# EricssonResearch/Robust-Tracking-MPC-over-Lossy-Networks

Hardware: AMD Instinct MI355X
Metric: QP solves/sec (= MPC steps/sec) at batch (higher is better)
Workload: dtype f64

## Files before the change

include/tmpc.h:

```cpp
#ifndef TMPC_H
#define TMPC_H

#include <stddef.h>
#include <stdint.h>

#ifdef __cplusplus
extern "C" {
#endif

#define TMPC_ABI_VERSION 5

#define TMPC_OK            0
#define TMPC_E_INVALID    -1
#define TMPC_E_UNSUPPORTED -2
#define TMPC_E_DEVICE     -3
#define TMPC_E_NOMEM      -4

#define TMPC_STATUS_OPTIMAL     0
#define TMPC_STATUS_MAX_ITER    1
#define TMPC_STATUS_INFEASIBLE  2
#define TMPC_STATUS_NUMERICAL   3
#define TMPC_STATUS_UNBOUNDED   4

typedef struct tmpc_problem {
// ... 128 lines not shown
                         int32_t *not_optimal, int32_t *overrun, int32_t *age_max, int64_t *age_sum, int32_t *iters_max, int64_t *iters_sum,
                         double *e_sum, double *e_max, double *e_q, float *kernel_ms);
int tmpc_series_stats(int device, int64_t B, int32_t T, const double *e, const uint32_t *word, int32_t G, const int32_t *group, int32_t n_q,
                      const double *q, int32_t *n_alive, int32_t *n_nan, int32_t *lost_up, int32_t *lost_down, int32_t *adopted, int32_t *tube,
                      int32_t *not_optimal, int32_t *overrun, int32_t *age_max, int64_t *age_sum, int32_t *iters_max, int64_t *iters_sum,
                      double *e_sum, double *e_max, double *e_q, float *kernel_ms);
int tmpc_mc_get_physics_error(tmpc_handle *h, int64_t B, double *err2_phys);

#define TMPC_ACTUATOR_CONSISTENT 0
#define TMPC_ACTUATOR_SMART      1
int tmpc_mc_set_actuator(tmpc_handle *h, int kind);

int tmpc_synchronize(tmpc_handle *h);

int tmpc_set_call_overlap(tmpc_handle *h, int on);
int tmpc_debug_lane_counters(tmpc_handle *h, int64_t *calls_per_lane, int64_t *cross_lane_waits, int reset);
int tmpc_debug_calls_conflict(int32_t nx, int32_t nu, int32_t N, int64_t B_a, const void *const *a, int64_t B_b, const void *const *b);

int tmpc_last_kernel_ms(tmpc_handle *h, float *ms);

int tmpc_kernel_ms_total(tmpc_handle *h, float *total_ms, int32_t *launches, int reset);

int tmpc_get_dims(const tmpc_handle *h, int variant, int32_t *nv, int32_t *nc, int32_t *npar);
int tmpc_get_factoring(const tmpc_handle *h, int variant, int32_t *nd, int32_t *ncc, int32_t *kc);

int tmpc_get_condensed(const tmpc_handle *h, int variant,
                       double *H, double *F1, double *F2, double *G, double *g0, double *E);

int tmpc_lp_batch(int device, int32_t d, int32_t nr, const double *H, const double *h,
                  int64_t B, const double *C, const int32_t *relax, double relax_by,
                  double *val, double *x, int32_t *status, int32_t *iters);
// ... 82 lines not shown
```

robust-tracking-mpc-over-lossy-networks_amd/LinearMPCOverNetworks/_native.py:

```python
from __future__ import annotations

import ctypes as C
import os

import numpy as np

_PKG = os.path.dirname(os.path.dirname(os.path.abspath(__file__)))
LIB_PATH = os.environ.get("TMPC_LIB") or os.path.join(_PKG, "lib", "libtmpc_hip.so")
ABI_VERSION = 5

_PTR_FIELDS = ["A", "B", "Q", "R", "P", "T", "K", "K_anc",
               "Hx", "hx", "Hu", "hu", "HT", "hT", "HZ", "hZ", "HZW", "hZW", "HTP", "hTP"]
_INT_FIELDS = ["nx", "nu", "N", "rx", "ru", "rT", "rZ", "rZW",
               "fixed_x0", "extended", "literal_terminal_row", "max_iter"]

_dp = C.POINTER(C.c_double)
_ip = C.POINTER(C.c_int32)
_up = C.POINTER(C.c_uint8)


class TmpcProblem(C.Structure):
    _fields_ = ([(n, C.c_int32) for n in _INT_FIELDS] + [("tol", C.c_double)]
                + [(n, _dp) for n in _PTR_FIELDS] + [("rTP", C.c_int32), ("terminal_equality", C.c_int32)])

# ... 133 lines not shown
        L.tmpc_lp_batch.restype = C.c_int
        L.tmpc_order_statistics.argtypes = [C.c_int, C.c_int64, C.c_int32, C.c_void_p, C.c_int32, C.c_void_p, C.c_void_p, C.c_void_p]
        L.tmpc_order_statistics.restype = C.c_int
        L.tmpc_estimate_w.argtypes = ([C.c_int, C.c_int32, C.c_int32] + [C.c_void_p] * 3 + [C.c_int, C.c_void_p, C.c_int32, C.c_int64, C.c_int32]
                                      + [C.c_void_p] * 3 + [C.c_uint64, C.c_int64, C.c_int32, C.c_void_p, C.c_double] + [C.c_void_p] * 10)
        L.tmpc_estimate_w.restype = C.c_int
        L.tmpc_estimate_w_models.argtypes = ([C.c_int, C.c_int32, C.c_int32] + [C.c_void_p] * 3 + [C.c_int, C.c_void_p, C.c_void_p, C.c_int32, C.c_int64, C.c_int32]
                                             + [C.c_void_p] * 3 + [C.c_uint64, C.c_int64, C.c_int32, C.c_void_p, C.c_double] + [C.c_void_p] * 10)
        L.tmpc_estimate_w_models.restype = C.c_int
        L.tmpc_synchronize.argtypes = [C.c_void_p]
        L.tmpc_synchronize.restype = C.c_int
        L.tmpc_set_call_overlap.argtypes = [C.c_void_p, C.c_int]
        L.tmpc_set_call_overlap.restype = C.c_int
        L.tmpc_debug_lane_counters.argtypes = [C.c_void_p, C.POINTER(C.c_int64), C.POINTER(C.c_int64), C.c_int]
        L.tmpc_debug_lane_counters.restype = C.c_int
        L.tmpc_debug_calls_conflict.argtypes = [C.c_int32, C.c_int32, C.c_int32, C.c_int64, C.POINTER(C.c_void_p), C.c_int64, C.POINTER(C.c_void_p)]
        L.tmpc_debug_calls_conflict.restype = C.c_int
        L.tmpc_last_kernel_ms.argtypes = [C.c_void_p, C.POINTER(C.c_float)]
        L.tmpc_last_kernel_ms.restype = C.c_int
        L.tmpc_kernel_ms_total.argtypes = [C.c_void_p, C.POINTER(C.c_float), _ip, C.c_int]
        L.tmpc_kernel_ms_total.restype = C.c_int
        L.tmpc_get_dims.argtypes = [C.c_void_p, C.c_int, _ip, _ip, _ip]
        L.tmpc_get_dims.restype = C.c_int
        L.tmpc_get_factoring.argtypes = [C.c_void_p, C.c_int, _ip, _ip, _ip]
        L.tmpc_get_factoring.restype = C.c_int
        L.tmpc_get_condensed.argtypes = [C.c_void_p, C.c_int, _dp, _dp, _dp, _dp, _dp, _dp]
        L.tmpc_get_condensed.restype = C.c_int
        L.tmpc_create_regulator.argtypes = [C.POINTER(TmpcRegulatorProblem), C.c_int, C.POINTER(C.c_void_p)]
        L.tmpc_create_regulator.restype = C.c_int
        L.tmpc_reg_run.argtypes = ([C.c_void_p, C.c_int64, C.c_int32] + [C.c_void_p] * 4 + [C.c_int32] + [C.c_void_p] * 2
# ... 233 lines not shown
        raise RuntimeError(h.error())


def set_call_overlap(h: Handle, on: bool = True):
    if lib().tmpc_set_call_overlap(h.ptr, int(bool(on))) != 0:
        raise RuntimeError(h.error())


def lane_counters(h: Handle, reset: bool = False):
    calls, waits = (C.c_int64 * 2)(), C.c_int64()
    if lib().tmpc_debug_lane_counters(h.ptr, calls, C.byref(waits), int(reset)) != 0:
        raise RuntimeError(h.error())
    return (int(calls[0]), int(calls[1])), int(waits.value)


SOLVE_POINTERS = ("x_k", "ref", "variant", "u_nom", "x_nom0", "xu_ss", "x_nom", "status", "iters")


def calls_conflict(nx: int, nu: int, N: int, B_a: int, a: dict, B_b: int, b: dict) -> bool:
    pa = (C.c_void_p * 9)(*[a.get(k) for k in SOLVE_POINTERS])
    pb = (C.c_void_p * 9)(*[b.get(k) for k in SOLVE_POINTERS])
    rc = lib().tmpc_debug_calls_conflict(nx, nu, N, int(B_a), pa, int(B_b), pb)
    if rc < 0:
        raise RuntimeError("tmpc_debug_calls_conflict: invalid argument")
    return bool(rc)


def last_kernel_ms(h: Handle) -> float:
    ms = C.c_float()
    if lib().tmpc_last_kernel_ms(h.ptr, C.byref(ms)) != 0:
# ... 942 lines not shown
```

robust-tracking-mpc-over-lossy-networks_amd/csrc/tmpc_api.cpp:

```cpp
#include "tmpc_host.hpp"

using namespace tmpc_host;

namespace {

constexpr size_t LANE_SPARE_EVENTS = 64;

template <class T>
int upload(tmpc_handle *h, Variant &v, const T *src, size_t n, const T **dst) {
    void *p = nullptr;
    if (h->device < 0) {
        p = std::malloc((n ? n : 1) * sizeof(T));
        if (!p) { h->err = "out of memory"; return TMPC_E_NOMEM; }
        v.dev.push_back(p);
        v.dev_bytes.push_back(n * sizeof(T));
        if (n) std::memcpy(p, src, n * sizeof(T));
        *dst = static_cast<const T *>(p);
        return TMPC_OK;
    }
    HIP_TRY(h, hipMalloc(&p, (n ? n : 1) * sizeof(T)));
    v.dev.push_back(p);
    v.dev_bytes.push_back(n * sizeof(T));
    if (n) HIP_TRY(h, hipMemcpy(p, src, n * sizeof(T), hipMemcpyHostToDevice));
    *dst = static_cast<const T *>(p);
// ... 274 lines not shown
}

int upload_variant(tmpc_handle *h, Variant &v, const tmpc_problem &p) {
    int rc;
    if ((rc = upload_wave(h, v, p))) return rc;
    if ((rc = upload_block(h, v, p))) return rc;
    if (!v.wave_ok && v.tiles == 0) {
        char buf[200];
        std::snprintf(buf, sizeof buf, "condensed QP (nv=%d, rows=%d) is outside the compiled kernels (nv <= 128)", v.c.nv, v.c.nc);
        h->err = buf;
        return TMPC_E_UNSUPPORTED;
    }
    return TMPC_OK;
}

int join_lanes(tmpc_handle *h) {
    Lane &second = h->lane[1];
    if (second.stream && !second.inflight.empty()) HIP_TRY(h, hipStreamWaitEvent(h->stream, second.inflight.back().end, 0));
    h->cur = 0;
    return TMPC_OK;
}

int ensure_block_ws(tmpc_handle *h, Lane &lane) {
    if (lane.blk_ws.p) return TMPC_OK;
    int ncp = 0, occ_max = 1;
    for (int k = 0; k < h->nvariants; ++k)
        if (h->v[k].tiles) { ncp = std::max(ncp, h->v[k].bq.ncp); occ_max = std::max(occ_max, tmpc::block_occupancy(h->v[k].tiles)); }
    h->blk_blocks = h->n_cu * occ_max;
    HIP_TRY(h, lane.blk_ws.reserve(static_cast<size_t>(h->blk_blocks) * tmpc::block_workspace_rows() * ncp * sizeof(double), lane.stream));
    return TMPC_OK;
}

size_t layout_staging(tmpc_handle *h, int64_t B) {
    const size_t nx = h->nx, nu = h->nu, N = h->N, b = static_cast<size_t>(B);
    auto up = [](size_t v) { return (v + 255) / 256 * 256; };
    h->off_r = up(b * nx * sizeof(double));
    h->off_var = h->off_r + up(b * nx * sizeof(double));
// ... 31 lines not shown
        h->stage_pin = nullptr;
        (void)hipGetLastError();
    }
    (void)layout_staging(h, B);
    return TMPC_OK;
}

int create_lane(tmpc_handle *h, Lane &lane) {
    HIP_TRY(h, hipStreamCreateWithFlags(&lane.stream, hipStreamNonBlocking));
    lane.wc.size = 4096;
    HIP_TRY(h, hipMalloc(reinterpret_cast<void **>(&lane.wc.ring), lane.wc.size * sizeof(unsigned long long)));
    HIP_TRY(h, hipMemset(lane.wc.ring, 0, lane.wc.size * sizeof(unsigned long long)));
    return TMPC_OK;
}

void prune_finished(Lane &lane) {
    while (!lane.inflight.empty()) {
        if (hipEventQuery(lane.inflight.front().end) != hipSuccess) { (void)hipGetLastError(); break; }
        lane.inflight.pop_front();
    }
}

bool conflicts_with_lane(const Lane &lane, const tmpc::CallRanges &call) {
    for (const Lane::InFlight &f : lane.inflight)
        if (tmpc::calls_conflict(f.touched, call)) return true;
    return false;
}

int pick_lane(tmpc_handle *h, const tmpc::CallRanges &call, Lane **out) {
    *out = &h->lane[0];
    if (!h->overlap) return TMPC_OK;
    for (Lane &l : h->lane) prune_finished(l);
    Lane &prev = h->lane[h->cur], &other = h->lane[1 - h->cur];
    if (conflicts_with_lane(prev, call)) {
        if (other.stream && conflicts_with_lane(other, call)) {
            HIP_TRY(h, hipStreamWaitEvent(prev.stream, other.inflight.back().end, 0));
            ++h->lane_waits;
        }
        *out = &prev;
        return TMPC_OK;
    }
    if (!other.stream) {
        if (prev.inflight.empty()) { *out = &prev; return TMPC_OK; }
        if (const int rc = create_lane(h, other)) return rc;
    }
    *out = &other;
    return TMPC_OK;
}

int note_in_flight(tmpc_handle *h, Lane &lane, const tmpc::CallRanges &call) {
    hipEvent_t end = h->ev1;
    if (h->pool_used >= 4096) {
        while (lane.inflight.size() >= LANE_SPARE_EVENTS) {
            HIP_TRY(h, hipEventSynchronize(lane.inflight.front().end));
            lane.inflight.pop_front();
        }
        if (lane.spare.size() < LANE_SPARE_EVENTS) {
            hipEvent_t e = nullptr;
            HIP_TRY(h, hipEventCreateWithFlags(&e, hipEventDisableTiming));
            lane.spare.push_back(e);
        }
        end = lane.spare[lane.spare_next++ % LANE_SPARE_EVENTS];
        HIP_TRY(h, hipEventRecord(end, lane.stream));
    }
    lane.inflight.push_back({call, end});
    ++lane.calls;
    h->cur = static_cast<int>(&lane - h->lane);
    return TMPC_OK;
}

int setup_handle(tmpc_handle *h, const tmpc_problem &p, int device) {
    if (device < 0) {
        for (int k = 0; k < h->nvariants; ++k) {
            const int rc = upload_variant(h, h->v[k], p);
            if (rc == TMPC_E_UNSUPPORTED) h->err.clear();
            else if (rc) return rc;
        }
        return TMPC_OK;
    }
    hipDeviceProp_t prop;
    hipError_t e = hipSetDevice(device);
    if (e == hipSuccess) e = hipGetDeviceProperties(&prop, device);
    if (e != hipSuccess) {
        h->err = std::string("tmpc_create: no usable HIP device: ") + hipGetErrorString(e);
        return TMPC_E_DEVICE;
    }
    h->n_cu = prop.multiProcessorCount;
    if (const int rc = create_lane(h, h->lane[0])) return rc;
    h->stream = h->lane[0].stream;
    for (int i = 0; i < 256; ++i) {
        hipEvent_t a = nullptr, b = nullptr;
        HIP_TRY(h, hipEventCreate(&a));
        HIP_TRY(h, hipEventCreate(&b));
        h->pool.emplace_back(a, b);
    }
    for (int k = 0; k < h->nvariants; ++k)
        if (const int rc = upload_variant(h, h->v[k], p)) return rc;
    return TMPC_OK;
}

template <class Condense>
int create_handle(const char *who, int nx, int nu, int N, int device, tmpc_handle **out, Condense condense) {
    *out = nullptr;
    if (nx <= 0 || nu <= 0 || N <= 0 || nx > 16) {
        g_create_error = std::string(who) + ": need 0 < nx <= 16, nu > 0, N > 0";
        return TMPC_E_INVALID;
    }
    tmpc_handle *h = new (std::nothrow) tmpc_handle();
    if (!h) { g_create_error = "out of memory"; return TMPC_E_NOMEM; }
    h->device = device; h->nx = nx; h->nu = nu; h->N = N;
    int rc = TMPC_E_INVALID;
    try {
// ... 46 lines not shown
                if (v.dev[i] == q) { n = v.dev_bytes[i]; break; }
        std::fwrite(&n, 8, 1, f);
        if (n) std::fwrite(q, 1, n, f);
    }
    std::fclose(f);
    return TMPC_OK;
}

}

namespace tmpc_host {

thread_local std::string g_create_error;

hipError_t sync_lanes(tmpc_handle *h) {
    hipError_t e = h->stream ? hipStreamSynchronize(h->stream) : hipSuccess;
    Lane &second = h->lane[1];
    if (e == hipSuccess && second.stream) e = hipStreamSynchronize(second.stream);
    if (e == hipSuccess)
        for (Lane &l : h->lane) l.inflight.clear();
    return e;
}

int pick_call_lane(tmpc_handle *h, const tmpc::CallRanges &call, Lane **out) { return pick_lane(h, call, out); }
int note_call(tmpc_handle *h, Lane &lane, const tmpc::CallRanges &call) { return h->overlap ? note_in_flight(h, lane, call) : (++lane.calls, TMPC_OK); }

bool use_block(const tmpc_handle *h, const Variant &v) { return h->kernel_path == TMPC_PATH_BLOCK ? v.tiles != 0 : !v.wave_ok; }

int ensure_reg_zero(tmpc_handle *h, int64_t B) {
    const size_t bytes = static_cast<size_t>(B) * h->nx * sizeof(double);
    if (bytes <= h->reg_zero.cap) return TMPC_OK;
    HIP_TRY(h, sync_lanes(h));
    HIP_TRY(h, h->reg_zero.reserve(bytes, h->stream));
    HIP_TRY(h, hipMemset(h->reg_zero.p, 0, bytes));
    return TMPC_OK;
}

int begin_timed_launch(tmpc_handle *h, Lane &lane) {
    hipEvent_t e0 = h->pool.back().first, e1 = h->pool.back().second;
    if (h->pool_used < 4096) {
// ... 161 lines not shown
}

int tmpc_solve_batch_device(tmpc_handle *h, int64_t B, const double *x_k, const double *ref, const uint8_t *variant,
                            double *u_nom, double *x_nom0, double *xu_ss, double *x_nom, int32_t *status, int32_t *iters) {
    if (const int rc = check_solve(h, "tmpc_solve_batch_device", B, x_k, ref, variant, u_nom, xu_ss, status, iters, false); rc || B == 0) return rc;
    if (h->regulator) {
        const int rz = ensure_reg_zero(h, B);
        if (rz) return rz;
        ref = h->reg_zero.as<double>();
    }
    const tmpc::CallRanges call = tmpc::solve_call_ranges(B, h->nx, h->nu, h->N, x_k, h->regulator ? nullptr : ref, variant, u_nom, x_nom0, xu_ss,
                                                          x_nom, status, iters);
    Lane *lane = nullptr;
    if (const int rc = pick_lane(h, call, &lane)) return rc;
    if (const int rc = enqueue(h, *lane, {B, x_k, ref, variant, u_nom, x_nom0, xu_ss, x_nom, status, iters})) return rc;
    return h->overlap ? note_in_flight(h, *lane, call) : (++lane->calls, TMPC_OK);
}

int tmpc_solve_batch(tmpc_handle *h, int64_t B, const double *x_k, const double *ref, const uint8_t *variant,
                     double *u_nom, double *x_nom0, double *xu_ss, double *x_nom, int32_t *status, int32_t *iters) {
    int rc = check_solve(h, "tmpc_solve_batch", B, x_k, ref, variant, u_nom, xu_ss, status, iters, true);
    if (rc || B == 0) return rc;
    if ((rc = join_lanes(h))) return rc;
    if ((rc = ensure_staging(h, B))) return rc;
    if (h->regulator && (rc = ensure_reg_zero(h, B))) return rc;
    const size_t nx = h->nx, nu = h->nu, N = h->N, b = static_cast<size_t>(B);
    const struct { size_t off; const void *host; size_t bytes; } in[] = {
        {0, x_k, b * nx * sizeof(double)}, {h->off_r, h->regulator ? nullptr : ref, b * nx * sizeof(double)}, {h->off_var, variant, b}};
    const struct { size_t off; void *host; size_t bytes; } out[] = {
        {0, u_nom, b * N * nu * sizeof(double)}, {h->off_x0, x_nom0, b * nx * sizeof(double)}, {h->off_ss, xu_ss, b * (nx + nu) * sizeof(double)},
        {h->off_st, status, b * sizeof(int32_t)}, {h->off_it, iters, b * sizeof(int32_t)}, {h->off_xn, x_nom, b * (N + 1) * nx * sizeof(double)}};
// ... 21 lines not shown
        if (a.host) HIP_TRY(h, hipMemcpyAsync(dev_in + a.off, a.host, a.bytes, hipMemcpyHostToDevice, h->stream));
    if ((rc = launch())) return rc;
    for (const auto &a : out)
        if (a.host) HIP_TRY(h, hipMemcpyAsync(a.host, dev_out + a.off, a.bytes, hipMemcpyDeviceToHost, h->stream));
    HIP_TRY(h, sync_lanes(h));
    return TMPC_OK;
}

int tmpc_set_kernel_path(tmpc_handle *h, int path) {
    if (!h || session_bars(h, "tmpc_set_kernel_path")) return TMPC_E_INVALID;
    if (path != TMPC_PATH_AUTO && path != TMPC_PATH_WAVE && path != TMPC_PATH_BLOCK) { h->err = "tmpc_set_kernel_path: unknown path"; return TMPC_E_INVALID; }
    for (int k = 0; k < h->nvariants; ++k) {
        if (path == TMPC_PATH_WAVE && !h->v[k].wave_ok && h->device >= 0) { h->err = "tmpc_set_kernel_path: no wave-per-QP shape covers this problem"; return TMPC_E_UNSUPPORTED; }
        if (path == TMPC_PATH_BLOCK && h->v[k].tiles == 0 && h->device >= 0) { h->err = "tmpc_set_kernel_path: the block kernel needs nv <= 128"; return TMPC_E_UNSUPPORTED; }
    }
    h->kernel_path = path;
    return TMPC_OK;
}

int tmpc_get_kernel_path(const tmpc_handle *h, int variant) {
    if (!h || variant < 0 || variant >= h->nvariants) return TMPC_E_INVALID;
    return use_block(h, h->v[variant]) ? TMPC_PATH_BLOCK : TMPC_PATH_WAVE;
}

int tmpc_debug_dump_layout(const tmpc_handle *h, int variant, const char *path) {
    if (!h || !path || variant < 0 || variant >= h->nvariants) return TMPC_E_INVALID;
    if (h->device >= 0) return TMPC_E_UNSUPPORTED;
    const Variant &v = h->v[variant];
    if (!v.wave_ok) return TMPC_E_UNSUPPORTED;
    const int32_t shp[6] = {v.shape.nvp, v.shape.dp, v.shape.ds, v.shape.kcp, v.shape.cp, v.shape.cs};
// ... 48 lines not shown

int tmpc_set_call_overlap(tmpc_handle *h, int on) {
    if (!h || session_bars(h, "tmpc_set_call_overlap")) return TMPC_E_INVALID;
    if (h->device >= 0 && (on != 0) != (h->overlap != 0)) {
        HIP_TRY(h, hipSetDevice(h->device));
        if (on) HIP_TRY(h, sync_lanes(h));
        else if (const int rc = join_lanes(h)) return rc;
    }
    h->overlap = on ? 1 : 0;
    return TMPC_OK;
}

int tmpc_debug_lane_counters(tmpc_handle *h, int64_t *calls_per_lane, int64_t *cross_lane_waits, int reset) {
    if (!h) return TMPC_E_INVALID;
    if (calls_per_lane)
        for (int k = 0; k < 2; ++k) calls_per_lane[k] = h->lane[k].calls;
    if (cross_lane_waits) *cross_lane_waits = h->lane_waits;
    if (reset) { h->lane[0].calls = h->lane[1].calls = 0; h->lane_waits = 0; }
    return TMPC_OK;
}

int tmpc_debug_calls_conflict(int32_t nx, int32_t nu, int32_t N, int64_t B_a, const void *const *a, int64_t B_b, const void *const *b) {
    if (!a || !b || nx <= 0 || nu <= 0 || N <= 0) return TMPC_E_INVALID;
    const tmpc::CallRanges ra = tmpc::solve_call_ranges(B_a, nx, nu, N, a[0], a[1], a[2], a[3], a[4], a[5], a[6], a[7], a[8]);
    const tmpc::CallRanges rb = tmpc::solve_call_ranges(B_b, nx, nu, N, b[0], b[1], b[2], b[3], b[4], b[5], b[6], b[7], b[8]);
    return tmpc::calls_conflict(ra, rb) ? 1 : 0;
}

int tmpc_last_kernel_ms(tmpc_handle *h, float *ms) {
    if (!h || !ms) return TMPC_E_INVALID;
    if (!h->timed) { h->err = "tmpc_last_kernel_ms: no solve has been enqueued yet"; return TMPC_E_INVALID; }
    HIP_TRY(h, hipEventSynchronize(h->ev1));
    HIP_TRY(h, hipEventElapsedTime(ms, h->ev0, h->ev1));
    return TMPC_OK;
}

int tmpc_kernel_ms_total(tmpc_handle *h, float *total_ms, int32_t *launches, int reset) {
    if (!h) return TMPC_E_INVALID;
    if (h->device < 0) { h->err = "host-only handle"; return TMPC_E_DEVICE; }
    HIP_TRY(h, sync_lanes(h));
    float sum = 0.f;
    size_t busy = 0;
    for (size_t i = 0; i < h->pool_used; ++i) {
        float ms = 0.f;
        HIP_TRY(h, hipEventElapsedTime(&ms, h->pool[i].first, h->pool[i].second));
        if (i > 0 && h->pool_lane[i] != h->pool_lane[busy]) {
            float past = 0.f;
            HIP_TRY(h, hipEventElapsedTime(&past, h->pool[busy].second, h->pool[i].second));
            if (past <= 0.f) continue;
            ms = std::min(ms, past);
        }
        busy = i;
        sum += ms;
    }
    if (total_ms) *total_ms = sum;
    if (launches) *launches = static_cast<int32_t>(h->pool_used);
    if (reset) h->pool_used = 0;
    return TMPC_OK;
}

#ifdef TMPC_STAMPS
int tmpc_debug_stamps(tmpc_handle *h, int variant, long long *out12 ) {
    if (!h || !out12) return TMPC_E_INVALID;
    HIP_TRY(h, sync_lanes(h));
    const long long *src = use_block(h, h->v[variant]) ? h->v[variant].db.dbg : h->v[variant].d.dbg;
    HIP_TRY(h, hipMemcpy(out12, src, 16 * sizeof(long long), hipMemcpyDeviceToHost));
    return TMPC_OK;
}
#endif
// ... 35 lines not shown
```

robust-tracking-mpc-over-lossy-networks_amd/csrc/tmpc_hazard.hpp:

```cpp
#pragma once
#include <cstddef>
#include <cstdint>

namespace tmpc {

struct ByteRange {
    uintptr_t lo = 0, hi = 0;
};

inline bool ranges_overlap(const ByteRange &a, const ByteRange &b) {
    return a.lo < a.hi && b.lo < b.hi && a.lo < b.hi && b.lo < a.hi;
}

struct CallRanges {
    static constexpr int NR = 8, NW = 8;
    ByteRange reads[NR], writes[NW];
    ByteRange hull;
};

inline ByteRange byte_range(const void *p, size_t bytes) {
    ByteRange r;
    if (p != nullptr && bytes != 0) { r.lo = reinterpret_cast<uintptr_t>(p); r.hi = r.lo + bytes; }
    return r;
}
// ... 21 lines not shown
    for (const ByteRange &r : c.writes) grow(r);
    return c;
}

inline bool calls_conflict(const CallRanges &earlier, const CallRanges &later) {
    if (!ranges_overlap(earlier.hull, later.hull)) return false;
    for (const ByteRange &w : earlier.writes) {
        for (const ByteRange &r : later.reads) if (ranges_overlap(w, r)) return true;
        for (const ByteRange &w2 : later.writes) if (ranges_overlap(w, w2)) return true;
    }
    for (const ByteRange &r : earlier.reads)
        for (const ByteRange &w2 : later.writes) if (ranges_overlap(r, w2)) return true;
    return false;
}

}
```

robust-tracking-mpc-over-lossy-networks_amd/csrc/tmpc_host.hpp:

```cpp
#pragma once
#include <hip/hip_runtime.h>

#include <cmath>
#include <cstdio>
#include <cstdlib>
#include <algorithm>
#include <cstdint>
#include <cstring>
#include <deque>
#include <initializer_list>
#include <new>
#include <string>
#include <vector>

#include "tmpc_condense.hpp"
#include "tmpc_device.hpp"
#include "tmpc_hazard.hpp"
#include "tmpc_law.hpp"

namespace tmpc_host __attribute__((visibility("hidden"))) {

struct DeviceBuffer {
    char *p = nullptr;
    size_t cap = 0;
// ... 59 lines not shown
    long long *tick_sum = nullptr, *tick_max = nullptr;
    int64_t tick_B = 0;
    double *err2_phys = nullptr;
    int64_t phys_B = 0;
    int fused = 0;
    std::vector<int32_t> link;
    int64_t link_B = 0;
    double *ser_e = nullptr;
    uint32_t *ser_w = nullptr;
    int64_t ser_B = 0;
    int ser_T = 0;
    tmpc::LawLoop law{};
    int64_t law_B = 0;
};

struct Lane {
    hipStream_t stream = nullptr;
    tmpc::WorkCounter wc;
    DeviceBuffer blk_ws;
    DeviceBuffer save;
    DeviceBuffer ticks;
    struct InFlight {
        tmpc::CallRanges touched;
        hipEvent_t end;
    };
    std::deque<InFlight> inflight;
    std::vector<hipEvent_t> spare;
    size_t spare_next = 0;
    int64_t calls = 0;
};

struct McSession {
    bool open = false, failed = false;
    int64_t B = 0;
    int T = 0, t = 0, extended = 0;
    tmpc::McModel m{};
    tmpc::McState st{};
    tmpc::McExternal ext{};
    int32_t *ws[2] = {nullptr, nullptr};
    bool warm = false;
    std::vector<double> ref;
    bool full_ref = false;
    double *ref_stage = nullptr;
    hipEvent_t ev_in = nullptr, ev_out = nullptr;
// ... 40 lines not shown
};
struct LawState;
struct SensState;
}

struct tmpc_handle {
    int device = 0;
    int n_cu = 0;
    int nvariants = 0;
    int nx = 0, nu = 0, N = 0;
    tmpc_host::Variant v[2];
    bool regulator = false;
    int reg_tube = 0;
    std::vector<double> hA, hB, hK, hKanc, hQ, hR;
    int kernel_path = TMPC_PATH_AUTO;
    tmpc_host::Lane lane[2];
    hipStream_t stream = nullptr;
    int overlap = 1;
    int cur = 0;
    int64_t lane_waits = 0;
    hipEvent_t ev0 = nullptr, ev1 = nullptr;
    bool timed = false;
    std::vector<std::pair<hipEvent_t, hipEvent_t>> pool;
    std::vector<uint8_t> pool_lane;
    size_t pool_used = 0;
    int blk_blocks = 0;
    int want_ticks = 0;
    int ticks_lane = 0;
    int64_t ticks_n = 0;
    tmpc_host::DeviceBuffer reg_zero;
    std::string err;
    tmpc_host::DeviceBuffer stage_dev;
    char *stage_pin = nullptr;
    size_t stage_in_bytes = 0, stage_out_bytes = 0, stage_out_core = 0;
// ... 18 lines not shown
            (h)->err = std::string(#expr) + ": " + hipGetErrorString(e_);                  \
            return TMPC_E_DEVICE;                                                          \
        }                                                                                  \
    } while (0)

extern thread_local std::string g_create_error;

hipError_t sync_lanes(tmpc_handle *h);
bool use_block(const tmpc_handle *h, const Variant &v);
int ensure_reg_zero(tmpc_handle *h, int64_t B);
int begin_timed_launch(tmpc_handle *h, Lane &lane);
int prepare_wave_scratch(tmpc_handle *h, Lane &lane, int64_t B, int nvar);
int enqueue(tmpc_handle *h, Lane &lane, const tmpc::BatchIO &io, int32_t *const *ws = nullptr, bool variants_valid = false);
void release_session(tmpc_handle *h);
int begin_loop(tmpc_handle *h, int64_t B);
bool session_bars(tmpc_handle *h, const char *who);
int pick_call_lane(tmpc_handle *h, const tmpc::CallRanges &call, Lane **out);
int note_call(tmpc_handle *h, Lane &lane, const tmpc::CallRanges &call);
void release_sens(tmpc_handle *h);
bool chol(std::vector<double> &a, int n);
void chol_solve(const std::vector<double> &L, int n, double *x);
std::string spd_inverse(const double *H, int n, std::vector<double> &Hinv);
struct HostModel {
    tmpc::Mat F, Eb, Y, Yp, Rec;
};
std::string host_model(const tmpc_handle *h, int k, HostModel &hm, int &rc);
int sens_signatures(tmpc_handle *h, const char *who, int64_t B, const double *x_k, const double *ref, const uint8_t *variant, const double *u_nom,
                    const double *x_nom0, const double *xu_ss, const int32_t *status, double act_tol, int32_t *flag, int32_t *n_active, uint32_t *active);
void release_law(tmpc_handle *h);
int enqueue_solves(tmpc_handle *h, Lane &lane, const tmpc::BatchIO &io, int32_t *const *ws);
// ... 6 lines not shown
```

robust-tracking-mpc-over-lossy-networks_amd/csrc/tmpc_law.cpp:

```cpp
#include <map>

#include "tmpc_host.hpp"
#include "tmpc_law.hpp"

using namespace tmpc_host;

namespace tmpc_host {

struct LawModel {
    int nv = 0, nc = 0, np = 0, ny = 0, npar = 0;
    std::vector<double> L, Ft, G, F, Eb, g0, Y, Yp, Ep, gp0;
    int nrow() const { return nc + npar; }
    int nrowp() const { return (nrow() + 63) / 64 * 64; }
    int nwords() const { return (nc + 31) / 32; }
};

struct LawRegion {
    std::vector<uint32_t> words;
    std::vector<double> S, K;
};

struct LawKeys {
    std::vector<unsigned long long> key;
    std::vector<int32_t> slot;
// ... 51 lines not shown
    }
    void release_device() {
        for (void *p : {static_cast<void *>(dS), static_cast<void *>(dK), static_cast<void *>(dorder), static_cast<void *>(dhits), static_cast<void *>(dkey),
                        static_cast<void *>(dslot)})
            if (p) (void)hipFree(p);
        dS = dK = nullptr; dorder = nullptr; dhits = nullptr; dkey = nullptr; dslot = nullptr; cap = 0;
    }
};

struct LawState {
    LawVariant v[2];
    double *dAB = nullptr;
    tmpc::LawTable *dtab = nullptr;
    int max_hops = 0;
    unsigned long long *dstats = nullptr;
    DeviceBuffer todo[2];
    DeviceBuffer stage;
};

void release_law(tmpc_handle *h) {
    LawState *s = h->law;
    if (!s) return;
    if (h->device >= 0) {
        for (LawVariant &v : s->v) v.release_device();
        if (s->dAB) (void)hipFree(s->dAB);
        if (s->dtab) (void)hipFree(s->dtab);
        if (s->dstats) (void)hipFree(s->dstats);
        for (DeviceBuffer &b : s->todo) b.release();
        s->stage.release();
    }
    delete s;
// ... 285 lines not shown
        for (int r = first_new; r < static_cast<int>(v.regions.size()); ++r) v.index.erase(v.regions[r].words);
        v.regions.resize(first_new);
        v.rebuild_keys();
        v.order.erase(std::remove_if(v.order.begin(), v.order.end(), [first_new](int32_t id) { return id >= first_new; }), v.order.end());
        for (int64_t i = 0; ids && i < n; ++i)
            if (ids[i] >= first_new) ids[i] = -1;
        if (n_new) *n_new = 0;
    }
    return rc;
}

int quiesce(tmpc_handle *h) {
    if (h->device < 0) return TMPC_OK;
    HIP_TRY(h, hipSetDevice(h->device));
    HIP_TRY(h, sync_lanes(h));
    h->cur = 0;
    return TMPC_OK;
}

struct LawCall {
    int64_t B;
    const double *x_k, *ref;
    const uint8_t *variant;
    const int32_t *hint;
    int max_tries;
    double *u_nom, *x_nom0, *xu_ss, *x_nom;
    int32_t *status, *iters, *region, *tries;
    bool fallback;
    const tmpc::LawLoop *loop = nullptr;
    const uint8_t *skip = nullptr;
    int32_t *const *ws = nullptr;
// ... 84 lines not shown
}

int call_device(tmpc_handle *h, const char *who, const LawCall &c) {
    if (const int rc = check_call(h, who, c); rc || c.B == 0) return rc;
    HIP_TRY(h, hipSetDevice(h->device));
    const tmpc::CallRanges call = law_call_ranges(h, c);
    Lane *lane = nullptr;
    if (const int rc = pick_call_lane(h, call, &lane)) return rc;
    if (const int rc = enqueue_law(h, *lane, who, c)) return rc;
    return note_call(h, *lane, call);
}

int call_host(tmpc_handle *h, const char *who, const LawCall &c) {
    if (const int rc = check_call(h, who, c); rc || c.B == 0) return rc;
    HIP_TRY(h, hipSetDevice(h->device));
    if (Lane &second = h->lane[1]; second.stream && !second.inflight.empty()) HIP_TRY(h, hipStreamWaitEvent(h->stream, second.inflight.back().end, 0));
    h->cur = 0;
    if (const int rc = ensure_state(h, who)) return rc;
    const size_t b = static_cast<size_t>(c.B), nx = h->nx, nu = h->nu, N = h->N, d = sizeof(double);
    struct Part { const void *host_in; void *host_out; size_t bytes; size_t off; };
    Part parts[] = {{c.x_k, nullptr, b * nx * d, 0}, {c.ref, nullptr, b * nx * d, 0}, {c.variant, nullptr, c.variant ? b : 0, 0}, {c.hint, nullptr, c.hint ? b * 4 : 0, 0},
                    {nullptr, c.u_nom, b * N * nu * d, 0}, {nullptr, c.x_nom0, b * nx * d, 0}, {nullptr, c.xu_ss, b * (nx + nu) * d, 0},
                    {nullptr, c.x_nom, c.x_nom ? b * (N + 1) * nx * d : 0, 0}, {nullptr, c.status, b * 4, 0}, {nullptr, c.iters, c.iters ? b * 4 : 0, 0},
                    {nullptr, c.region, b * 4, 0}, {nullptr, c.tries, c.tries ? b * 4 : 0, 0}};
    size_t total = 0;
    for (Part &p : parts) { p.off = total; total += (p.bytes + 255) / 256 * 256; }
    LawState &s = *h->law;
    HIP_TRY(h, s.stage.reserve(std::max<size_t>(total, 256), h->stream));
    char *base = s.stage.p;
    for (const Part &p : parts)
        if (p.host_in && p.bytes) HIP_TRY(h, hipMemcpyAsync(base + p.off, p.host_in, p.bytes, hipMemcpyHostToDevice, h->stream));
    auto at = [&](int i) { return parts[i].bytes ? base + parts[i].off : nullptr; };
// ... 349 lines not shown
```

robust-tracking-mpc-over-lossy-networks_amd/csrc/tmpc_sens.cpp:

```cpp
#include "tmpc_host.hpp"
#include "tmpc_sens.hpp"

using namespace tmpc_host;

namespace tmpc_host {

struct SensModel {
    bool ready = false;
    char *block = nullptr;
    tmpc::SensArgs a{};
};

struct SensState {
    SensModel m[2];
    DeviceBuffer ws[2];
    DeviceBuffer stage;
};

void release_sens(tmpc_handle *h) {
    SensState *s = h->sens;
    if (!s) return;
    for (SensModel &m : s->m)
        if (m.block) (void)hipFree(m.block);
    for (DeviceBuffer &b : s->ws) b.release();
    s->stage.release();
    delete s;
    h->sens = nullptr;
}

bool chol(std::vector<double> &a, int n) {
// ... 271 lines not shown
        a.nz0 = N * nu; a.nz1 = nx; a.nz2 = nx + nu;
        a.Z0 = c.u_nom; a.Z1 = c.x_nom0; a.Z2 = c.xu_ss;
        a.status = c.status; a.variant = c.variant; a.my_variant = k; a.nvariants = h->nvariants;
        a.act_tol = c.act_tol > 0.0 ? c.act_tol : tmpc::SENS_ACT_TOL;
        a.mode = c.mode; a.ybar = c.ybar; a.out = c.out; a.flag = c.flag; a.n_active = c.n_active; a.active = c.active;
        a.nwords = nwords_of(h);
        a.ws = c.mode == tmpc::SENS_MODE_JACOBIAN ? wsbuf.as<double>() : nullptr;
        HIP_TRY(h, tmpc::launch_sens(a, sens_blocks(c.B, h->n_cu, a.nv, a.np), lane.stream));
    }
    HIP_TRY(h, hipEventRecord(h->ev1, lane.stream));
    h->timed = true;
    return TMPC_OK;
}

int primary_behind_secondary(tmpc_handle *h) {
    Lane &second = h->lane[1];
    if (second.stream && !second.inflight.empty()) HIP_TRY(h, hipStreamWaitEvent(h->stream, second.inflight.back().end, 0));
    h->cur = 0;
    return TMPC_OK;
}

tmpc::CallRanges sens_call_ranges(const tmpc_handle *h, const SensCall &c) {
    const size_t b = static_cast<size_t>(c.B), nx = h->nx, nu = h->nu, N = h->N, ny = N * nu + 2 * nx + nu, d = sizeof(double);
    tmpc::CallRanges r;
    static_assert(tmpc::CallRanges::NR >= 8 && tmpc::CallRanges::NW >= 4, "eight arrays read, four written");
    r.reads[0] = tmpc::byte_range(c.x_k, b * nx * d);
    r.reads[1] = tmpc::byte_range(c.ref, b * nx * d);
    r.reads[2] = tmpc::byte_range(c.variant, b);
    r.reads[3] = tmpc::byte_range(c.u_nom, b * N * nu * d);
    r.reads[4] = tmpc::byte_range(c.x_nom0, b * nx * d);
    r.reads[5] = tmpc::byte_range(c.xu_ss, b * (nx + nu) * d);
    r.reads[6] = tmpc::byte_range(c.status, b * sizeof(int32_t));
    r.reads[7] = tmpc::byte_range(c.ybar, b * ny * d);
    r.writes[0] = tmpc::byte_range(c.out, b * (c.mode == tmpc::SENS_MODE_VJP ? 2 * nx : ny * 2 * nx) * d);
// ... 180 lines not shown
```

Measured before the change: 13.00 million.

## Generalize call overlap from two streams to up to four lanes

After: 13.28 million (median of 6 runs). 1.02x the previous value.

```diff
diff --git a/include/tmpc.h b/include/tmpc.h
--- a/include/tmpc.h
+++ b/include/tmpc.h
@@ -166,7 +166,16 @@
 int tmpc_synchronize(tmpc_handle *h);
 
 int tmpc_set_call_overlap(tmpc_handle *h, int on);
+#define TMPC_MAX_LANES 4
+int tmpc_set_call_lanes(tmpc_handle *h, int n);
+int tmpc_get_call_lanes(const tmpc_handle *h);
 int tmpc_debug_lane_counters(tmpc_handle *h, int64_t *calls_per_lane, int64_t *cross_lane_waits, int reset);
+int tmpc_debug_lane_counters_n(tmpc_handle *h, int64_t *calls_per_lane, int64_t *cross_lane_waits, int reset);
+int tmpc_debug_elastic_grid(const tmpc_handle *h, int32_t n_cu, int32_t lanes, int32_t wpb, int64_t B, int32_t *core, int32_t *eligible);
+int tmpc_debug_surplus_yields(uint32_t followers, int32_t lanes);
+int tmpc_debug_plan_lanes(int32_t nx, int32_t nu, int32_t N, int32_t lanes, int32_t n_calls, const int64_t *B, const void *const *ptrs,
+                          int32_t *lane_out, int32_t *waited_out, int32_t *followers_out);
+double tmpc_debug_busy_union(int32_t n, const int32_t *lane, const double *start, const double *end);
 int tmpc_debug_calls_conflict(int32_t nx, int32_t nu, int32_t N, int64_t B_a, const void *const *a, int64_t B_b, const void *const *b);
 
 int tmpc_last_kernel_ms(tmpc_handle *h, float *ms);
diff --git a/robust-tracking-mpc-over-lossy-networks_amd/LinearMPCOverNetworks/_native.py b/robust-tracking-mpc-over-lossy-networks_amd/LinearMPCOverNetworks/_native.py
--- a/robust-tracking-mpc-over-lossy-networks_amd/LinearMPCOverNetworks/_native.py
+++ b/robust-tracking-mpc-over-lossy-networks_amd/LinearMPCOverNetworks/_native.py
@@ -171,6 +171,22 @@
         L.tmpc_set_call_overlap.restype = C.c_int
         L.tmpc_debug_lane_counters.argtypes = [C.c_void_p, C.POINTER(C.c_int64), C.POINTER(C.c_int64), C.c_int]
         L.tmpc_debug_lane_counters.restype = C.c_int
+        if hasattr(L, "tmpc_set_call_lanes"):
+            L.tmpc_set_call_lanes.argtypes = [C.c_void_p, C.c_int]
+            L.tmpc_set_call_lanes.restype = C.c_int
+            L.tmpc_get_call_lanes.argtypes = [C.c_void_p]
+            L.tmpc_get_call_lanes.restype = C.c_int
+            L.tmpc_debug_lane_counters_n.argtypes = [C.c_void_p, C.POINTER(C.c_int64), C.POINTER(C.c_int64), C.c_int]
+            L.tmpc_debug_lane_counters_n.restype = C.c_int
+            L.tmpc_debug_elastic_grid.argtypes = [C.c_void_p, C.c_int32, C.c_int32, C.c_int32, C.c_int64, C.POINTER(C.c_int32), C.POINTER(C.c_int32)]
+            L.tmpc_debug_elastic_grid.restype = C.c_int
+            L.tmpc_debug_surplus_yields.argtypes = [C.c_uint32, C.c_int32]
+            L.tmpc_debug_surplus_yields.restype = C.c_int
+            L.tmpc_debug_plan_lanes.argtypes = [C.c_int32, C.c_int32, C.c_int32, C.c_int32, C.c_int32, C.POINTER(C.c_int64), C.POINTER(C.c_void_p),
+                                                C.POINTER(C.c_int32), C.POINTER(C.c_int32), C.POINTER(C.c_int32)]
+            L.tmpc_debug_plan_lanes.restype = C.c_int
+            L.tmpc_debug_busy_union.argtypes = [C.c_int32, C.POINTER(C.c_int32), C.POINTER(C.c_double), C.POINTER(C.c_double)]
+            L.tmpc_debug_busy_union.restype = C.c_double
         L.tmpc_debug_calls_conflict.argtypes = [C.c_int32, C.c_int32, C.c_int32, C.c_int64, C.POINTER(C.c_void_p), C.c_int64, C.POINTER(C.c_void_p)]
         L.tmpc_debug_calls_conflict.restype = C.c_int
         L.tmpc_last_kernel_ms.argtypes = [C.c_void_p, C.POINTER(C.c_float)]
@@ -434,6 +450,54 @@
     return (int(calls[0]), int(calls[1])), int(waits.value)
 
 
+MAX_LANES = 4
+
+
+def set_call_lanes(h: Handle, n: int):
+    if lib().tmpc_set_call_lanes(h.ptr, int(n)) != 0:
+        raise RuntimeError(h.error())
+
+
+def get_call_lanes(h: Handle) -> int:
+    return int(lib().tmpc_get_call_lanes(h.ptr))
+
+
+def lane_counters_n(h: Handle, reset: bool = False):
+    calls, waits = (C.c_int64 * MAX_LANES)(), C.c_int64()
+    if lib().tmpc_debug_lane_counters_n(h.ptr, calls, C.byref(waits), int(reset)) != 0:
+        raise RuntimeError(h.error())
+    return tuple(int(c) for c in calls), int(waits.value)
+
+
+def elastic_grid(h: Handle, n_cu: int, lanes: int, wpb: int, B: int):
+    core, el = C.c_int32(), C.c_int32()
+    if lib().tmpc_debug_elastic_grid(h.ptr, n_cu, lanes, wpb, int(B), C.byref(core), C.byref(el)) != 0:
+        raise RuntimeError("tmpc_debug_elastic_grid: invalid argument")
+    return int(core.value), bool(el.value)
+
+
+def surplus_yields(followers: int, lanes: int) -> bool:
+    return bool(lib().tmpc_debug_surplus_yields(int(followers), int(lanes)))
+
+
+def plan_lanes(nx: int, nu: int, N: int, lanes: int, calls):
+    n = len(calls)
+    B = (C.c_int64 * max(n, 1))(*[int(b) for b, _ in calls])
+    ptrs = (C.c_void_p * (9 * max(n, 1)))(*[a.get(k) for _, a in calls for k in SOLVE_POINTERS])
+    lane, waited, fol = ((C.c_int32 * max(n, 1))() for _ in range(3))
+    if lib().tmpc_debug_plan_lanes(nx, nu, N, int(lanes), n, B, ptrs, lane, waited, fol) != 0:
+        raise RuntimeError("tmpc_debug_plan_lanes: invalid argument")
+    return [(int(lane[i]), int(waited[i]), int(fol[i])) for i in range(n)]
+
+
+def busy_union(lanes, start, end) -> float:
+    n = len(lanes)
+    la = (C.c_int32 * max(n, 1))(*[int(x) for x in lanes])
+    s = (C.c_double * max(n, 1))(*[float(x) for x in start])
+    e = (C.c_double * max(n, 1))(*[float(x) for x in end])
+    return float(lib().tmpc_debug_busy_union(n, la, s, e))
+
+
 SOLVE_POINTERS = ("x_k", "ref", "variant", "u_nom", "x_nom0", "xu_ss", "x_nom", "status", "iters")
 
 
diff --git a/robust-tracking-mpc-over-lossy-networks_amd/csrc/tmpc_api.cpp b/robust-tracking-mpc-over-lossy-networks_amd/csrc/tmpc_api.cpp
--- a/robust-tracking-mpc-over-lossy-networks_amd/csrc/tmpc_api.cpp
+++ b/robust-tracking-mpc-over-lossy-networks_amd/csrc/tmpc_api.cpp
@@ -312,13 +312,6 @@
     return TMPC_OK;
 }
 
-int join_lanes(tmpc_handle *h) {
-    Lane &second = h->lane[1];
-    if (second.stream && !second.inflight.empty()) HIP_TRY(h, hipStreamWaitEvent(h->stream, second.inflight.back().end, 0));
-    h->cur = 0;
-    return TMPC_OK;
-}
-
 int ensure_block_ws(tmpc_handle *h, Lane &lane) {
     if (lane.blk_ws.p) return TMPC_OK;
     int ncp = 0, occ_max = 1;
@@ -380,6 +373,8 @@
     return TMPC_OK;
 }
 
+int lanes_in_use(const tmpc_handle *h) { return h->overlap ? std::min(h->lanes, max_lanes(h)) : 1; }
+
 void prune_finished(Lane &lane) {
     while (!lane.inflight.empty()) {
         if (hipEventQuery(lane.inflight.front().end) != hipSuccess) { (void)hipGetLastError(); break; }
@@ -395,23 +390,37 @@
 
 int pick_lane(tmpc_handle *h, const tmpc::CallRanges &call, Lane **out) {
     *out = &h->lane[0];
-    if (!h->overlap) return TMPC_OK;
-    for (Lane &l : h->lane) prune_finished(l);
-    Lane &prev = h->lane[h->cur], &other = h->lane[1 - h->cur];
-    if (conflicts_with_lane(prev, call)) {
-        if (other.stream && conflicts_with_lane(other, call)) {
-            HIP_TRY(h, hipStreamWaitEvent(prev.stream, other.inflight.back().end, 0));
-            ++h->lane_waits;
-        }
-        *out = &prev;
-        return TMPC_OK;
-    }
-    if (!other.stream) {
-        if (prev.inflight.empty()) { *out = &prev; return TMPC_OK; }
-        if (const int rc = create_lane(h, other)) return rc;
-    }
-    *out = &other;
-    return TMPC_OK;
+    const int n = lanes_in_use(h);
+    if (n <= 1) return TMPC_OK;
+    tmpc::LaneView view[tmpc::MAX_LANES];
+    for (int l = 0; l < n; ++l) {
+        Lane &lane = h->lane[l];
+        if (!lane.active) continue;
+        prune_finished(lane);
+        view[l].exists = true;
+        view[l].busy = !lane.inflight.empty();
+        view[l].conflicts = conflicts_with_lane(lane, call);
+    }
+    const tmpc::LanePick pick = tmpc::pick_lane_policy(view, n, h->cur);
+    Lane &lane = h->lane[pick.lane];
+    if (pick.create) {
+        if (!lane.stream)
+            if (const int rc = create_lane(h, lane)) return rc;
+        lane.active = true;
+    }
+    for (int l = 0; l < n; ++l)
+        if (pick.wait_mask >> l & 1u) HIP_TRY(h, hipStreamWaitEvent(lane.stream, h->lane[l].inflight.back().end, 0));
+    if (pick.wait_mask) ++h->lane_waits;
+    *out = &lane;
+    return TMPC_OK;
+}
+
+void count_call(tmpc_handle *h, Lane &lane) {
+    const int idx = static_cast<int>(&lane - h->lane);
+    if (idx != h->cur) h->par ^= 1;
+    ++h->par_calls[h->par];
+    ++lane.calls;
+    h->cur = idx;
 }
 
 int note_in_flight(tmpc_handle *h, Lane &lane, const tmpc::CallRanges &call) {
@@ -430,9 +439,13 @@
         HIP_TRY(h, hipEventRecord(end, lane.stream));
     }
     lane.inflight.push_back({call, end});
-    ++lane.calls;
-    h->cur = static_cast<int>(&lane - h->lane);
-    return TMPC_OK;
+    count_call(h, lane);
+    return TMPC_OK;
+}
+
+void read_lane_settings(tmpc_handle *h) {
+    h->lanes = DEFAULT_CALL_LANES;
+    if (const char *e = std::getenv("TMPC_CALL_LANES")) h->lanes = std::min(std::max(std::atoi(e), 1), tmpc::MAX_LANES);
 }
 
 int setup_handle(tmpc_handle *h, const tmpc_problem &p, int device) {
@@ -442,6 +455,7 @@
             if (rc == TMPC_E_UNSUPPORTED) h->err.clear();
             else if (rc) return rc;
         }
+        read_lane_settings(h);
         return TMPC_OK;
     }
     hipDeviceProp_t prop;
@@ -453,6 +467,7 @@
     }
     h->n_cu = prop.multiProcessorCount;
     if (const int rc = create_lane(h, h->lane[0])) return rc;
+    h->lane[0].active = true;
     h->stream = h->lane[0].stream;
     for (int i = 0; i < 256; ++i) {
         hipEvent_t a = nullptr, b = nullptr;
@@ -462,6 +477,9 @@
     }
     for (int k = 0; k < h->nvariants; ++k)
         if (const int rc = upload_variant(h, h->v[k], p)) return rc;
+    read_lane_settings(h);
+    for (int l = 1; l < std::min(h->lanes, max_lanes(h)); ++l)
+        if (const int rc = create_lane(h, h->lane[l])) return rc;
     return TMPC_OK;
 }
 
@@ -538,16 +556,31 @@
 thread_local std::string g_create_error;
 
 hipError_t sync_lanes(tmpc_handle *h) {
-    hipError_t e = h->stream ? hipStreamSynchronize(h->stream) : hipSuccess;
-    Lane &second = h->lane[1];
-    if (e == hipSuccess && second.stream) e = hipStreamSynchronize(second.stream);
+    hipError_t e = hipSuccess;
+    for (Lane &l : h->lane)
+        if (e == hipSuccess && l.stream) e = hipStreamSynchronize(l.stream);
     if (e == hipSuccess)
         for (Lane &l : h->lane) l.inflight.clear();
     return e;
 }
 
+int join_lanes(tmpc_handle *h) {
+    for (int l = 1; l < tmpc::MAX_LANES; ++l) {
+        Lane &other = h->lane[l];
+        if (other.stream && !other.inflight.empty()) HIP_TRY(h, hipStreamWaitEvent(h->stream, other.inflight.back().end, 0));
+    }
+    h->cur = h->par = 0;
+    return TMPC_OK;
+}
+
+int max_lanes(const tmpc_handle *h) {
+    for (int k = 0; k < h->nvariants; ++k)
+        if (use_block(h, h->v[k])) return 2;
+    return tmpc::MAX_LANES;
+}
+
 int pick_call_lane(tmpc_handle *h, const tmpc::CallRanges &call, Lane **out) { return pick_lane(h, call, out); }
-int note_call(tmpc_handle *h, Lane &lane, const tmpc::CallRanges &call) { return h->overlap ? note_in_flight(h, lane, call) : (++lane.calls, TMPC_OK); }
+int note_call(tmpc_handle *h, Lane &lane, const tmpc::CallRanges &call) { return lanes_in_use(h) > 1 ? note_in_flight(h, lane, call) : (count_call(h, lane), TMPC_OK); }
 
 bool use_block(const tmpc_handle *h, const Variant &v) { return h->kernel_path == TMPC_PATH_BLOCK ? v.tiles != 0 : !v.wave_ok; }
 
@@ -739,7 +772,7 @@
     Lane *lane = nullptr;
     if (const int rc = pick_lane(h, call, &lane)) return rc;
     if (const int rc = enqueue(h, *lane, {B, x_k, ref, variant, u_nom, x_nom0, xu_ss, x_nom, status, iters})) return rc;
-    return h->overlap ? note_in_flight(h, *lane, call) : (++lane->calls, TMPC_OK);
+    return lanes_in_use(h) > 1 ? note_in_flight(h, *lane, call) : (count_call(h, *lane), TMPC_OK);
 }
 
 int tmpc_solve_batch(tmpc_handle *h, int64_t B, const double *x_k, const double *ref, const uint8_t *variant,
@@ -791,6 +824,11 @@
         if (path == TMPC_PATH_WAVE && !h->v[k].wave_ok && h->device >= 0) { h->err = "tmpc_set_kernel_path: no wave-per-QP shape covers this problem"; return TMPC_E_UNSUPPORTED; }
         if (path == TMPC_PATH_BLOCK && h->v[k].tiles == 0 && h->device >= 0) { h->err = "tmpc_set_kernel_path: the block kernel needs nv <= 128"; return TMPC_E_UNSUPPORTED; }
     }
+    if (h->device >= 0 && path != h->kernel_path) {
+        HIP_TRY(h, hipSetDevice(h->device));
+        HIP_TRY(h, sync_lanes(h));
+        h->cur = h->par = 0;
+    }
     h->kernel_path = path;
     return TMPC_OK;
 }
@@ -869,10 +907,84 @@
 int tmpc_debug_lane_counters(tmpc_handle *h, int64_t *calls_per_lane, int64_t *cross_lane_waits, int reset) {
     if (!h) return TMPC_E_INVALID;
     if (calls_per_lane)
-        for (int k = 0; k < 2; ++k) calls_per_lane[k] = h->lane[k].calls;
+        for (int k = 0; k < 2; ++k) calls_per_lane[k] = h->par_calls[k];
     if (cross_lane_waits) *cross_lane_waits = h->lane_waits;
-    if (reset) { h->lane[0].calls = h->lane[1].calls = 0; h->lane_waits = 0; }
-    return TMPC_OK;
+    if (reset) {
+        for (tmpc_host::Lane &l : h->lane) l.calls = 0;
+        h->par_calls[0] = h->par_calls[1] = 0;
+        h->lane_waits = 0;
+    }
+    return TMPC_OK;
+}
+
+int tmpc_debug_lane_counters_n(tmpc_handle *h, int64_t *calls_per_lane, int64_t *cross_lane_waits, int reset) {
+    if (!h) return TMPC_E_INVALID;
+    if (calls_per_lane)
+        for (int l = 0; l < tmpc::MAX_LANES; ++l) calls_per_lane[l] = h->lane[l].calls;
+    return tmpc_debug_lane_counters(h, nullptr, cross_lane_waits, reset);
+}
+
+int tmpc_set_call_lanes(tmpc_handle *h, int n) {
+    if (!h || session_bars(h, "tmpc_set_call_lanes")) return TMPC_E_INVALID;
+    if (n < 1 || n > tmpc::MAX_LANES) { h->err = "tmpc_set_call_lanes: 1 ... TMPC_MAX_LANES lanes"; return TMPC_E_INVALID; }
+    if (h->device >= 0 && n != h->lanes) {
+        HIP_TRY(h, hipSetDevice(h->device));
+        HIP_TRY(h, sync_lanes(h));
+        h->cur = h->par = 0;
+    }
+    h->lanes = n;
+    return TMPC_OK;
+}
+
+int tmpc_get_call_lanes(const tmpc_handle *h) { return h ? (h->overlap ? std::min(h->lanes, max_lanes(h)) : 1) : TMPC_E_INVALID; }
+
+int tmpc_debug_elastic_grid(const tmpc_handle *h, int32_t n_cu, int32_t lanes, int32_t wpb, int64_t B, int32_t *core, int32_t *eligible) {
+    if (!h || n_cu <= 0 || lanes < 1 || lanes > tmpc::MAX_LANES || wpb <= 0) return TMPC_E_INVALID;
+    const bool block_variant = max_lanes(h) < tmpc::MAX_LANES;
+    const int l = std::min<int>(lanes, max_lanes(h));
+    if (core) *core = tmpc::elastic_core(n_cu, l);
+    if (eligible) *eligible = tmpc::elastic_eligible(B, n_cu, wpb, block_variant) && tmpc::elastic_core(n_cu, l) < n_cu ? 1 : 0;
+    return TMPC_OK;
+}
+
+int tmpc_debug_surplus_yields(uint32_t followers, int32_t lanes) { return tmpc::surplus_yields(followers, lanes) ? 1 : 0; }
+
+int tmpc_debug_plan_lanes(int32_t nx, int32_t nu, int32_t N, int32_t lanes, int32_t n_calls, const int64_t *B, const void *const *ptrs,
+                          int32_t *lane_out, int32_t *waited_out, int32_t *followers_out) {
+    if (!B || !ptrs || !lane_out || nx <= 0 || nu <= 0 || N <= 0 || n_calls < 0 || lanes < 1 || lanes > tmpc::MAX_LANES) return TMPC_E_INVALID;
+    std::vector<tmpc::CallRanges> calls;
+    std::vector<int> held[tmpc::MAX_LANES];
+    std::vector<int32_t> fol(static_cast<size_t>(n_calls), 0);
+    bool exists[tmpc::MAX_LANES] = {true, false, false, false};
+    int cur = 0;
+    for (int i = 0; i < n_calls; ++i) {
+        const void *const *a = ptrs + static_cast<size_t>(i) * 9;
+        calls.push_back(tmpc::solve_call_ranges(B[i], nx, nu, N, a[0], a[1], a[2], a[3], a[4], a[5], a[6], a[7], a[8]));
+        tmpc::LaneView view[tmpc::MAX_LANES];
+        for (int l = 0; l < lanes; ++l) {
+            view[l].exists = exists[l];
+            view[l].busy = !held[l].empty();
+            for (int j : held[l]) view[l].conflicts = view[l].conflicts || tmpc::calls_conflict(calls[j], calls[i]);
+        }
+        const tmpc::LanePick pick = tmpc::pick_lane_policy(view, lanes, cur);
+        exists[pick.lane] = true;
+        const unsigned beside = tmpc::follower_lanes(pick, view, lanes);
+        for (int l = 0; l < lanes; ++l)
+            if (beside >> l & 1u)
+                for (int j : held[l]) ++fol[j];
+        held[pick.lane].push_back(i);
+        cur = pick.lane;
+        lane_out[i] = pick.lane;
+        if (waited_out) waited_out[i] = static_cast<int32_t>(pick.wait_mask);
+    }
+    if (followers_out) std::copy(fol.begin(), fol.end(), followers_out);
+    return TMPC_OK;
+}
+
+double tmpc_debug_busy_union(int32_t n, const int32_t *lane, const double *start, const double *end) {
+    if (n < 0 || !lane || !start || !end) return -1.0;
+    return tmpc::busy_union(static_cast<size_t>(n), [&](size_t i, double *ms) { *ms = end[i] - start[i]; return true; },
+                            [&](size_t j, size_t i, double *ms) { *ms = end[i] - end[j]; return true; }, [&](size_t i) { return lane[i]; });
 }
 
 int tmpc_debug_calls_conflict(int32_t nx, int32_t nu, int32_t N, int64_t B_a, const void *const *a, int64_t B_b, const void *const *b) {
@@ -894,20 +1006,14 @@
     if (!h) return TMPC_E_INVALID;
     if (h->device < 0) { h->err = "host-only handle"; return TMPC_E_DEVICE; }
     HIP_TRY(h, sync_lanes(h));
-    float sum = 0.f;
-    size_t busy = 0;
-    for (size_t i = 0; i < h->pool_used; ++i) {
-        float ms = 0.f;
-        HIP_TRY(h, hipEventElapsedTime(&ms, h->pool[i].first, h->pool[i].second));
-        if (i > 0 && h->pool_lane[i] != h->pool_lane[busy]) {
-            float past = 0.f;
-            HIP_TRY(h, hipEventElapsedTime(&past, h->pool[busy].second, h->pool[i].second));
-            if (past <= 0.f) continue;
-            ms = std::min(ms, past);
-        }
-        busy = i;
-        sum += ms;
-    }
+    hipError_t bad = hipSuccess;
+    bool ok = true;
+    const float sum = static_cast<float>(tmpc::busy_union(
+        h->pool_used,
+        [&](size_t i, double *ms) { float t = 0.f; bad = hipEventElapsedTime(&t, h->pool[i].first, h->pool[i].second); *ms = t; return bad == hipSuccess; },
+        [&](size_t j, size_t i, double *ms) { float t = 0.f; bad = hipEventElapsedTime(&t, h->pool[j].second, h->pool[i].second); *ms = t; return bad == hipSuccess; },
+        [&](size_t i) { return h->pool_lane[i]; }, &ok));
+    if (!ok) HIP_TRY(h, bad);
     if (total_ms) *total_ms = sum;
     if (launches) *launches = static_cast<int32_t>(h->pool_used);
     if (reset) h->pool_used = 0;
diff --git a/robust-tracking-mpc-over-lossy-networks_amd/csrc/tmpc_hazard.hpp b/robust-tracking-mpc-over-lossy-networks_amd/csrc/tmpc_hazard.hpp
--- a/robust-tracking-mpc-over-lossy-networks_amd/csrc/tmpc_hazard.hpp
+++ b/robust-tracking-mpc-over-lossy-networks_amd/csrc/tmpc_hazard.hpp
@@ -59,4 +59,79 @@
     return false;
 }
 
+
+constexpr int MAX_LANES = 4;
+
+struct LaneView {
+    bool exists = false, busy = false, conflicts = false;
+};
+struct LanePick {
+    int lane = 0;
+    bool create = false;
+    unsigned wait_mask = 0;
+};
+
+inline LanePick pick_lane_policy(const LaneView *v, int lanes, int cur) {
+    LanePick p;
+    if (lanes <= 1) return p;
+    if (cur < 0 || cur >= lanes) cur = 0;
+    int target = -1;
+    if (v[cur].exists && v[cur].conflicts) target = cur;
+    for (int k = 1; k < lanes && target < 0; ++k) {
+        const int l = (cur + k) % lanes;
+        if (v[l].exists && v[l].conflicts) target = l;
+    }
+    if (target < 0) {
+        target = (cur + 1) % lanes;
+        if (!v[target].exists) {
+            bool all_busy = true;
+            for (int l = 0; l < lanes; ++l)
+                if (v[l].exists && !v[l].busy) all_busy = false;
+            if (all_busy) p.create = true;
+            else target = target == 1 ? cur : 0;
+        }
+    }
+    p.lane = target;
+    for (int l = 0; l < lanes; ++l)
+        if (l != target && v[l].exists && v[l].conflicts) p.wait_mask |= 1u << l;
+    return p;
 }
+
+inline int elastic_core(int n_cu, int lanes) {
+    if (n_cu < 1) return 1;
+    if (lanes <= 2) return n_cu;
+    return (n_cu + lanes - 2) / (lanes - 1);
+}
+inline bool elastic_eligible(int64_t B, int n_cu, int wpb, bool block_variant) {
+    return !block_variant && n_cu > 0 && wpb > 0 && B >= 2 * static_cast<int64_t>(n_cu) * wpb;
+}
+inline bool surplus_yields(unsigned followers, int lanes) { return lanes >= 2 && followers >= static_cast<unsigned>(lanes - 1); }
+inline unsigned follower_lanes(const LanePick &p, const LaneView *v, int lanes) {
+    unsigned m = 0;
+    if (p.wait_mask != 0) return 0;
+    for (int l = 0; l < lanes; ++l)
+        if (l != p.lane && v[l].exists && v[l].busy) m |= 1u << l;
+    return m;
+}
+
+template <class Own, class Past, class LaneOf>
+inline double busy_union(size_t n, Own own, Past past, LaneOf lane, bool *ok = nullptr) {
+    double sum = 0.0;
+    size_t busy = 0;
+    if (ok) *ok = true;
+    for (size_t i = 0; i < n; ++i) {
+        double ms = 0.0;
+        if (!own(i, &ms)) { if (ok) *ok = false; return sum; }
+        if (i > 0 && lane(i) != lane(busy)) {
+            double p = 0.0;
+            if (!past(busy, i, &p)) { if (ok) *ok = false; return sum; }
+            if (p <= 0.0) continue;
+            if (p < ms) ms = p;
+        }
+        busy = i;
+        sum += ms;
+    }
+    return sum;
+}
+
+}
diff --git a/robust-tracking-mpc-over-lossy-networks_amd/csrc/tmpc_host.hpp b/robust-tracking-mpc-over-lossy-networks_amd/csrc/tmpc_host.hpp
--- a/robust-tracking-mpc-over-lossy-networks_amd/csrc/tmpc_host.hpp
+++ b/robust-tracking-mpc-over-lossy-networks_amd/csrc/tmpc_host.hpp
@@ -97,6 +97,8 @@
     int64_t law_B = 0;
 };
 
+constexpr int DEFAULT_CALL_LANES = 3;
+
 struct Lane {
     hipStream_t stream = nullptr;
     tmpc::WorkCounter wc;
@@ -111,6 +113,7 @@
     std::vector<hipEvent_t> spare;
     size_t spare_next = 0;
     int64_t calls = 0;
+    bool active = false;
 };
 
 struct McSession {
@@ -181,10 +184,13 @@
     int reg_tube = 0;
     std::vector<double> hA, hB, hK, hKanc, hQ, hR;
     int kernel_path = TMPC_PATH_AUTO;
-    tmpc_host::Lane lane[2];
+    tmpc_host::Lane lane[tmpc::MAX_LANES];
     hipStream_t stream = nullptr;
     int overlap = 1;
+    int lanes = 2;
     int cur = 0;
+    int par = 0;
+    int64_t par_calls[2] = {0, 0};
     int64_t lane_waits = 0;
     hipEvent_t ev0 = nullptr, ev1 = nullptr;
     bool timed = false;
@@ -233,6 +239,8 @@
 int enqueue(tmpc_handle *h, Lane &lane, const tmpc::BatchIO &io, int32_t *const *ws = nullptr, bool variants_valid = false);
 void release_session(tmpc_handle *h);
 int begin_loop(tmpc_handle *h, int64_t B);
+int join_lanes(tmpc_handle *h);
+int max_lanes(const tmpc_handle *h);
 bool session_bars(tmpc_handle *h, const char *who);
 int pick_call_lane(tmpc_handle *h, const tmpc::CallRanges &call, Lane **out);
 int note_call(tmpc_handle *h, Lane &lane, const tmpc::CallRanges &call);
diff --git a/robust-tracking-mpc-over-lossy-networks_amd/csrc/tmpc_law.cpp b/robust-tracking-mpc-over-lossy-networks_amd/csrc/tmpc_law.cpp
--- a/robust-tracking-mpc-over-lossy-networks_amd/csrc/tmpc_law.cpp
+++ b/robust-tracking-mpc-over-lossy-networks_amd/csrc/tmpc_law.cpp
@@ -89,7 +89,7 @@
     tmpc::LawTable *dtab = nullptr;
     int max_hops = 0;
     unsigned long long *dstats = nullptr;
-    DeviceBuffer todo[2];
+    DeviceBuffer todo[tmpc::MAX_LANES];
     DeviceBuffer stage;
 };
 
@@ -405,7 +405,7 @@
     if (h->device < 0) return TMPC_OK;
     HIP_TRY(h, hipSetDevice(h->device));
     HIP_TRY(h, sync_lanes(h));
-    h->cur = 0;
+    h->cur = h->par = 0;
     return TMPC_OK;
 }
 
@@ -520,8 +520,7 @@
 int call_host(tmpc_handle *h, const char *who, const LawCall &c) {
     if (const int rc = check_call(h, who, c); rc || c.B == 0) return rc;
     HIP_TRY(h, hipSetDevice(h->device));
-    if (Lane &second = h->lane[1]; second.stream && !second.inflight.empty()) HIP_TRY(h, hipStreamWaitEvent(h->stream, second.inflight.back().end, 0));
-    h->cur = 0;
+    if (const int rc = join_lanes(h)) return rc;
     if (const int rc = ensure_state(h, who)) return rc;
     const size_t b = static_cast<size_t>(c.B), nx = h->nx, nu = h->nu, N = h->N, d = sizeof(double);
     struct Part { const void *host_in; void *host_out; size_t bytes; size_t off; };
diff --git a/robust-tracking-mpc-over-lossy-networks_amd/csrc/tmpc_sens.cpp b/robust-tracking-mpc-over-lossy-networks_amd/csrc/tmpc_sens.cpp
--- a/robust-tracking-mpc-over-lossy-networks_amd/csrc/tmpc_sens.cpp
+++ b/robust-tracking-mpc-over-lossy-networks_amd/csrc/tmpc_sens.cpp
@@ -13,7 +13,7 @@
 
 struct SensState {
     SensModel m[2];
-    DeviceBuffer ws[2];
+    DeviceBuffer ws[tmpc::MAX_LANES];
     DeviceBuffer stage;
 };
 
@@ -315,10 +315,7 @@
 }
 
 int primary_behind_secondary(tmpc_handle *h) {
-    Lane &second = h->lane[1];
-    if (second.stream && !second.inflight.empty()) HIP_TRY(h, hipStreamWaitEvent(h->stream, second.inflight.back().end, 0));
-    h->cur = 0;
-    return TMPC_OK;
+    return join_lanes(h);
 }
 
 tmpc::CallRanges sens_call_ranges(const tmpc_handle *h, const SensCall &c) {
```
